# DevSinghSachan/emdr2

Measured on AMD Instinct MI355X. Metric: mips_queries_per_sec, higher is better.
Workload: dtype f16; 1 GPU; BASELINE configs[1]: MIPS-only top-50, 512 queries/search over a 21015324 x 768 fp16 index resident in HBM; rows=21015324, dim=768, top_k=50, parallelism=index row-sharded x1, all-gather(top-k) + merge, cus=256, allgather_bytes_per_rank=0

## Files before the change

### emdr2_amd/_native.py

```python
import ctypes
import os

_HERE = os.path.dirname(os.path.abspath(__file__))
LIB_PATH = os.path.join(_HERE, "lib", "libemdr2_hip.so")

EMDR2_ABI_VERSION = 4
FLAG_AMBIGUOUS = 1
FLAG_OVERFLOW = 2
MAX_TOPK = 120

_ERRORS = {-1: "bad argument", -2: "workspace too small", -3: "HIP launch/runtime error", -4: "unsupported shape"}

_vp, _i32, _i64, _sz = ctypes.c_void_p, ctypes.c_int, ctypes.c_int64, ctypes.c_size_t
SIGNATURES = {
    "emdr2_abi_version": (_i32, []),
    "emdr2_device_cu_count": (_i32, []),
    "emdr2_mips_layout_bytes": (_i32, [_i64, _i32, ctypes.POINTER(_sz)]),
    "emdr2_mips_pack_rows": (_i32, [_vp, _i64, _i32, _i64, _i64, _vp, _vp, _vp]),
    "emdr2_mips_unpack_rows": (_i32, [_vp, _i64, _i32, _vp, _i64, _vp, _vp]),
    "emdr2_mips_workspace_bytes": (_i32, [_i32, _i32, _i32, ctypes.POINTER(_sz)]),
    "emdr2_mips_search": (_i32, [_vp, _i64, _i32, _i64, _vp, _vp, _i32, _i32, _vp, _vp, _vp, _vp, _vp, _vp, _sz, _vp]),
    "emdr2_mips_exact_workspace_bytes": (_i32, [_i64, _i32, ctypes.POINTER(_sz)]),
    "emdr2_mips_search_exact": (_i32, [_vp, _i64, _i32, _i64, _vp, _i32, _vp, _i32, _i32, _vp, _vp, _vp, _vp, _vp, _vp, _sz, _vp]),
    "emdr2_mips_merge": (_i32, [_vp, _vp, _vp, _i32, _i32, _i32, _vp, _vp, _vp, _vp]),
    "emdr2_mips_search_f32": (_i32, [_vp, _i64, _i32, _i64, _vp, _vp, _i32, _i32, _vp, _vp, _vp, _vp, _vp, _vp, _sz, _vp]),
    "emdr2_mips_exact_workspace_bytes_f32": (_i32, [_i64, _i32, ctypes.POINTER(_sz)]),
    "emdr2_mips_search_exact_f32": (_i32, [_vp, _i64, _i32, _i64, _vp, _i32, _vp, _i32, _i32, _vp, _vp, _vp, _vp, _vp, _vp, _sz, _vp]),
    "emdr2_mips_merge_f32": (_i32, [_vp, _vp, _vp, _i32, _i32, _i32, _vp, _vp, _vp, _vp]),
    "emdr2_mips_search_records": (_i32, [_vp, _i64, _i32, _i64, _vp, _vp, _i32, _i32, _vp, _i32, _vp, _vp, _vp, _sz, _vp]),
    "emdr2_mips_merge_records": (_i32, [_vp, _i32, _i32, _i32, _i32, _vp, _vp, _vp, _vp]),
    "emdr2_mips_pack_records": (_i32, [_vp, _vp, _vp, _vp, _i32, _i32, _i32, _vp, _vp]),
    "emdr2_mips_shadow_bytes": (_i32, [_i64, _i32, ctypes.POINTER(_sz), ctypes.POINTER(_sz)]),
    "emdr2_mips_seal_shadow": (_i32, [_vp, _i64, _i32, _vp, _vp, _vp, _vp]),
    "emdr2_mips_search_shadow": (_i32, [_vp, _i64, _i32, _i64, _vp, _vp, _vp, _i64, _vp, _i32, _i32, _vp, _i32, _vp, _vp, _vp, _vp, _vp, _vp, _sz, _vp]),
    "emdr2_mips_shadow_launches": (_i32, []),
    "emdr2_mips_debug_scores": (_i32, [_vp, _i64, _i32, _vp, _i32, _vp, _vp, _sz, _vp]),
    "emdr2_mips_set_timing": (_i32, [_i32]),
    "emdr2_mips_timing_collect": (_i32, [ctypes.POINTER(ctypes.c_float), ctypes.POINTER(_i64), _i32, ctypes.POINTER(_i32)]),
}

SIGNATURES["emdr2_assemble_evidence"] = (_i32, [_vp, _vp, _i32, _i32, _i32, _vp, _vp, _i32, _vp, _i32, _i32, _i32, _i32, _i32,
                                                  _vp, _vp, _vp, _vp, _vp, _vp])


_f32 = ctypes.c_float
_u32 = ctypes.c_uint32
SIGNATURES["emdr2_gemm_nt_bf16"] = (_i32, [_vp, _i64, _vp, _i64, _vp, _i64, _i32, _i32, _i32, _i32, _i64, _i64, _i64, _i32, _i64, _i64, _i64,
                                             _f32, _vp, _i32, _vp, _vp, _i32, _i32, _i32, _f32, _u32, _vp])
SIGNATURES["emdr2_gemm_tn_bf16"] = (_i32, [_vp, _i64, _vp, _i64, _vp, _i64, _i32, _i32, _i32, _i32, _vp, _vp])
SIGNATURES["emdr2_dropout"] = (_i32, [_vp, _vp, _i64, _i32, _f32, _u32, _vp])
SIGNATURES["emdr2_transpose_bf16"] = (_i32, [_vp, _i64, _vp, _i64, _i32, _i32, _i32, _i64, _i64, _i32, _i64, _i64, _vp, _vp])


SIGNATURES.update({
    "emdr2_layernorm_fwd": (_i32, [_vp, _vp, _vp, _vp, _vp, _vp, _i64, _i32, _f32, _vp]),
    "emdr2_layernorm_bwd": (_i32, [_vp, _vp, _vp, _vp, _vp, _vp, _vp, _vp, _vp, _i64, _i32, _vp]),
    "emdr2_layernorm_bwd_mask": (_i32, [_vp, _vp, _vp, _vp, _vp, _vp, _vp, _vp, _vp, _i64, _i32, _vp, _f32, _u32, _vp]),
    "emdr2_softmax_mask_fwd": (_i32, [_vp, _vp, _vp, _i32, _i32, _i32, _i32, _i32, _vp, _vp, _f32, _u32, _vp]),
    "emdr2_softmax_mask_bwd": (_i32, [_vp, _vp, _vp, _vp, _vp, _vp, _i32, _i32, _i32, _i32, _i32, _f32, _u32, _vp, _vp]),
    "emdr2_softmax_mask_t": (_i32, [_vp, _vp, _vp, _vp, _vp, _vp, _vp, _i32, _i32, _i32, _i32, _i32, _f32, _u32, _vp]),
    "emdr2_gelu_bwd": (_i32, [_vp, _vp, _vp, _i64, _vp]),
    "emdr2_embedding_fwd": (_i32, [_vp, _vp, _vp, _vp, _vp, _vp, _i64, _i32, _i32, _f32, _u32, _vp]),
    "emdr2_embedding_bwd": (_i32, [_vp, _vp, _vp, _vp, _vp, _vp, _i64, _i32, _i32, _i32, _f32, _u32, _vp]),
    "emdr2_attention_fwd": (_i32, [_vp, _i64, _i64, _i64, _vp, _i64, _i64, _i64, _vp, _i64, _i64, _i64, _vp, _vp, _vp, _i32, _i32, _i32, _i32, _i32, _i32,
                                   _f32, _f32, _u32, _vp, _vp, _vp]),
    "emdr2_attention_bwd": (_i32, [_vp, _i64, _i64, _i64, _vp, _i64, _i64, _i64, _vp, _i64, _i64, _i64, _vp, _vp, _vp, _i64, _i64, _vp, _vp, _i64, _i64,
                                   _vp, _vp, _vp, _vp, _vp, _i32, _i32, _i32, _i32, _i32, _i32, _f32, _f32, _u32, _vp]),
    "emdr2_lse_gather_fwd": (_i32, [_vp, _vp, _vp, _vp, _i64, _i32, _vp]),
    "emdr2_lse_gather_bwd": (_i32, [_vp, _vp, _vp, _vp, _vp, _i64, _i32, _vp]),
    "emdr2_sumsq_f32": (_i32, [_vp, _i64, _vp, _vp, _vp]),
    "emdr2_adam_step": (_i32, [_vp, _vp, _vp, _vp, _vp, _i64, _f32, _f32, _f32, _f32, _f32, _i32, _vp, _f32, _vp]),
    "emdr2_adam_step_flat": (_i32, [_vp, _vp, _vp, _vp, _vp, _i64, _i64, _f32, _f32, _f32, _f32, _f32, _i32, _vp, _f32, _vp]),
    "emdr2_scale_cast_f32_to_bf16": (_i32, [_vp, _vp, _i64, _f32, _vp]),
    "emdr2_widen_bf16_to_f32": (_i32, [_vp, _vp, _i64, _vp]),
    "emdr2_cast_f32_to_bf16": (_i32, [_vp, _vp, _i64, _vp]),
    "emdr2_accum_bf16_to_f32": (_i32, [_vp, _vp, _i64, _f32, _vp]),
})


SIGNATURES.update({
    "emdr2_seq_lengths": (_i32, [_vp, _i32, _i32, _vp, _vp, _vp]),
    "emdr2_seq_pack_ids": (_i32, [_vp, _vp, _vp, _i32, _i32, _i64, _i64, _vp, _vp, _vp, _vp, _vp]),
    "emdr2_gather_rows": (_i32, [_vp, _vp, _vp, _i64, _i32, _vp]),
    "emdr2_scatter_rows": (_i32, [_vp, _vp, _vp, _i64, _i32, _vp]),
    "emdr2_embedding_packed_fwd": (_i32, [_vp, _vp, _vp, _vp, _vp, _vp, _vp, _i64, _i32, _i32, _f32, _u32, _vp]),
    "emdr2_embedding_packed_bwd": (_i32, [_vp, _vp, _vp, _i32, _vp, _vp, _vp, _vp, _i64, _i32, _i32, _i32, _f32, _u32, _vp]),
    "emdr2_attention_varlen_fwd": (_i32, [_vp, _i64, _i64, _i64, _vp, _i64, _i64, _i64, _vp, _i64, _i64, _i64, _vp, _vp, _vp, _vp, _vp, _i64, _i64,
                                          _i32, _i32, _i32, _i32, _i32, _i32, _f32, _f32, _u32, _vp, _vp, _vp]),
# ... 77 lines not shown
```

### emdr2_amd/csrc/mips_api.hip

```cpp
#include "../../include/emdr2_mips.h"
#include "mips_kernels.h"
#include "exp_hooks.h"
#include <stdlib.h>

namespace {

#define TIMING_SLOTS 2048
struct Timing {
    bool enabled = false;
    hipEvent_t ev[2 * TIMING_SLOTS] = {};
    int created = 0;
    int n = 0;
    int64_t rows[TIMING_SLOTS] = {};
} g_timing;

int cu_count()
{
    static int cus = 0;
    if (!cus) {
        int dev = 0;
        hipDeviceProp_t prop;
        if (hipGetDevice(&dev) != hipSuccess || hipGetDeviceProperties(&prop, dev) != hipSuccess) return 256;
        cus = prop.multiProcessorCount > 0 ? prop.multiProcessorCount : 256;
    }
    return cus;
}

inline size_t align_up(size_t x, size_t a) { return (x + a - 1) / a * a; }

#define env_int(name, dflt) EXP_ENV_INT(name, dflt)

struct Workspace {
    char *q_frag;
    char *q_tiled;
    float *qnorm, *tau;
    unsigned *count;
    uint2 *cand, *cand8;
};

size_t carve(char *base, int dim, Workspace *w)
{
    size_t off = 0;
    auto take = [&](size_t bytes) { char *p = base ? base + off : nullptr; off += align_up(bytes, 256); return p; };
    char *f = take((size_t)(dim / 32) * 512 * 64);
    char *a = take((size_t)(dim / 32) * 512 * 64);
    char *b = take(512 * sizeof(float));
    char *c = take(512 * sizeof(float));
    char *d = take((512 + 8 * 512 + 8 * (size_t)SCAN8_PROG_UINTS) * sizeof(unsigned));
    char *e = take((size_t)512 * CAPQ * sizeof(uint2));
    char *g = take((size_t)512 * 8 * SUBCAP * sizeof(uint2));
    if (w) { w->q_frag = f; w->q_tiled = a; w->qnorm = (float *)b; w->tau = (float *)c; w->count = (unsigned *)d; w->cand = (uint2 *)e; w->cand8 = (uint2 *)g; }
    return off;
}

struct Shadow {
    const void *image;
    const float *table;
    int64_t min_rows;
};
long g_shadow_launches = 0;

bool bad_shape(int64_t n_rows, int dim) { return n_rows < 0 || n_rows >= ((int64_t)1 << 31) - 1024 || dim < 64 || dim > 8192 || (dim % 32) != 0; }

}

extern "C" {

int emdr2_abi_version(void) { return EMDR2_ABI_VERSION; }

int emdr2_device_cu_count(void) { return cu_count(); }

int emdr2_mips_set_timing(int enabled)
{
    g_timing.enabled = enabled != 0;
    g_timing.n = 0;
    return EMDR2_OK;
}

int emdr2_mips_timing_collect(float *ms, int64_t *rows, int max_n, int *n_out)
{
    const int n = g_timing.n < max_n ? g_timing.n : max_n;
    for (int i = 0; i < n; ++i) {
        if (hipEventSynchronize(g_timing.ev[2 * i + 1]) != hipSuccess) return EMDR2_E_LAUNCH;
        if (hipEventElapsedTime(&ms[i], g_timing.ev[2 * i], g_timing.ev[2 * i + 1]) != hipSuccess) return EMDR2_E_LAUNCH;
        rows[i] = g_timing.rows[i];
    }
    if (n_out) *n_out = n;
    g_timing.n = 0;
    return EMDR2_OK;
}

int emdr2_mips_layout_bytes(int64_t n_rows, int dim, size_t *bytes)
{
    if (!bytes || bad_shape(n_rows, dim)) return EMDR2_E_BADARG;
    const int64_t padded = (n_rows + 511) / 512 * 512;
    *bytes = (size_t)padded * dim * 2;
    return EMDR2_OK;
}

int emdr2_mips_pack_rows(const void *rows_rm, int64_t n_chunk, int dim, int64_t row_offset, int64_t n_rows_total,
                         void *tiled, float *emax_sq, emdr2_stream_t stream)
{
    if (!rows_rm || !tiled || !emax_sq || bad_shape(n_rows_total, dim) || n_chunk < 0 || row_offset < 0 ||
        row_offset + n_chunk > n_rows_total)
        return EMDR2_E_BADARG;
    return mips_launch_pack_rows(rows_rm, n_chunk, dim, row_offset, tiled, emax_sq, (hipStream_t)stream);
}

int emdr2_mips_unpack_rows(const void *tiled, int64_t n_rows_total, int dim, const int64_t *row_ids, int64_t n_out,
                           void *rows_rm, emdr2_stream_t stream)
{
    if (!tiled || !row_ids || !rows_rm || bad_shape(n_rows_total, dim) || n_out < 0) return EMDR2_E_BADARG;
    return mips_launch_unpack_rows(tiled, dim, row_ids, n_out, rows_rm, (hipStream_t)stream);
}

int emdr2_mips_workspace_bytes(int n_q, int dim, int k, size_t *bytes)
{
    if (!bytes || n_q < 1 || k < 1 || k > EMDR2_MAX_TOPK || bad_shape(0, dim)) return EMDR2_E_BADARG;
    *bytes = carve(nullptr, dim, nullptr);
    return EMDR2_OK;
}

static int variant_for(int nq) { return nq <= 128 ? 2 : (nq <= 256 ? 1 : 0); }
static const int kBM[3] = {128, 256, 512};
static const int kBN[3] = {512, 256, 128};

static int search_impl(const void *tiled, int64_t n_rows, int dim, int64_t row_base, const float *emax_sq,
                       const void *queries, int n_q, int k, const int32_t *ids, void *out_dist, int32_t *out_idx,
                       int64_t *out_row, uint32_t *out_flags, void *workspace, size_t workspace_bytes,
                       emdr2_stream_t stream_, int f32, uint4 *out_rec = nullptr, const Shadow *shadow = nullptr)
{
    if (!tiled || !emax_sq || !queries || !out_flags || !workspace) return EMDR2_E_BADARG;
    if (!out_rec && (!out_dist || !out_idx || !out_row)) return EMDR2_E_BADARG;
    if (out_rec && ((uintptr_t)out_rec & 15)) return EMDR2_E_BADARG;
    if (n_q < 1 || k < 1 || k > EMDR2_MAX_TOPK || bad_shape(n_rows, dim) || n_rows < 1) return EMDR2_E_BADARG;
    Workspace w;
    if (carve((char *)workspace, dim, &w) > workspace_bytes) return EMDR2_E_WORKSPACE;
    hipStream_t stream = (hipStream_t)stream_;
    const int kp = k <= 56 ? 64 : 128;
    const int seg0 = env_int("EMDR2_MIPS_SEG0", 8192) / 512 * 512;
    const int growth = env_int("EMDR2_MIPS_GROWTH", 8);
    const int growth_i8 = env_int("EMDR2_MIPS_GROWTH_I8", 2);
    if (seg0 < 512 || seg0 > (int)CAPQ - 512 || growth < 2 || growth_i8 < 2) return EMDR2_E_BADARG;
    const int force_variant = env_int("EMDR2_MIPS_VARIANT", -1);
    const int cus = env_int("EMDR2_MIPS_GRID", cu_count());
    const int scan_kernel = env_int("EMDR2_MIPS_KERNEL", 1);
    const int ablate = env_int("EMDR2_MIPS_ABLATE", 0);

    for (int q0 = 0; q0 < n_q; q0 += EMDR2_MAX_QUERIES_PER_PASS) {
        const int nqp = (n_q - q0) < EMDR2_MAX_QUERIES_PER_PASS ? (n_q - q0) : EMDR2_MAX_QUERIES_PER_PASS;
        int variant = variant_for(nqp);
        if (force_variant >= 0 && force_variant <= 2 && kBN[force_variant] >= nqp) variant = force_variant;
        const int BM = kBM[variant], BN = kBN[variant];
        const uint16_t *qp = (const uint16_t *)queries + (size_t)q0 * dim;
        int rc;
        if ((rc = mips_launch_pack_queries(qp, nqp, dim, BN, w.q_tiled, w.qnorm, stream))) return rc;
        EXP_MIPS_PACK_QUERIES_FRAG(variant, scan_kernel, qp, nqp, dim, w, stream, rc)
        const int64_t dense_rows = n_rows < seg0 ? n_rows : seg0;
        unsigned *const count8 = w.count + 512, *const prog0 = count8 + 8 * 512;
        if ((rc = mips_launch_init(w.tau, w.count, out_flags + q0, BN, nqp, (unsigned)dense_rows, count8,
                                   8 * 512 + (variant == 0 ? 8 * (size_t)SCAN8_PROG_UINTS : 0), stream)))
            return rc;

        ScanParams sp;
        sp.e_tiled = (const char *)tiled;
        sp.q_tiled = w.q_tiled;
        sp.tau = w.tau;
        sp.cand = w.cand;
        sp.count = w.count;
        sp.flags = out_flags + q0;
        sp.dense_out = nullptr;
        sp.nch = dim / 32;
        sp.n_rows = (int)n_rows;
        sp.n_q = nqp;
        sp.capq = CAPQ;
        sp.cand8 = w.cand8;
        sp.count8 = count8;
        sp.dense_row0 = 0;
        sp.tune = env_int("EMDR2_MIPS_TUNE", 17);
        sp.trace = (unsigned long long *)w.cand + (size_t)511 * CAPQ;

        int scan8_launches = 0;
        const bool shadow_ok = shadow && variant <= 1 && scan_kernel == 1 && (dim % 256) == 0 && n_rows - dense_rows >= shadow->min_rows;
        char *const q8_tiled = w.q_frag;
        float *const qc = (float *)(w.q_frag + (size_t)(dim / 64) * 512 * 64);
        if (shadow_ok && (rc = mips_launch_pack_queries_i8(qp, nqp, dim, BN, q8_tiled, qc, stream))) return rc;
        const bool couple = EXP_MIPS_COUPLE();
        int64_t done = 0, seg_end = dense_rows;
        int mode = 1;
        while (done < n_rows) {
            sp.tile_begin = (int)(done / BM);
            sp.tile_end = (int)((seg_end + BM - 1) / BM);
            const int tiles = sp.tile_end - sp.tile_begin;
            const int grid = tiles < cus ? tiles : cus;
            const bool timed = g_timing.enabled && g_timing.n < TIMING_SLOTS;
            if (timed) {
                while (g_timing.created <= g_timing.n) {
                    if (hipEventCreate(&g_timing.ev[2 * g_timing.created]) != hipSuccess ||
                        hipEventCreate(&g_timing.ev[2 * g_timing.created + 1]) != hipSuccess)
                        return EMDR2_E_LAUNCH;
                    ++g_timing.created;
                }
                if (hipEventRecord(g_timing.ev[2 * g_timing.n], stream) != hipSuccess) return EMDR2_E_LAUNCH;
            }
            bool int8_segment = false;
            EXP_MIPS_SCAN_VARIANT(mode, variant, ablate, scan_kernel, sp, w, grid, seg_end, n_rows, done, stream, rc)
            {
                rc = -4;
                if (mode == 0 && variant <= 1 && scan_kernel == 1) {
                    unsigned *prog = (couple && scan8_launches < 8) ? prog0 + (size_t)SCAN8_PROG_UINTS * scan8_launches : nullptr;
                    if (shadow_ok && seg_end - done >= shadow->min_rows) {
                        rc = mips_launch_scan8i(sp, shadow->image, shadow->table, q8_tiled, qc, BN, done, seg_end, cus, prog, stream);
                        if (rc == 0) { int8_segment = true; ++g_shadow_launches; }
                    }
                    if (rc == -4) rc = mips_launch_scan8(sp, BN, done, seg_end, cus, prog, stream);
                    if (rc == 0) ++scan8_launches;
                }
                if (rc == -4) rc = mips_launch_scan(variant, mode, sp, grid, stream);
            }
            if (rc) return rc;
            if (timed) {
                if (hipEventRecord(g_timing.ev[2 * g_timing.n + 1], stream) != hipSuccess) return EMDR2_E_LAUNCH;
                g_timing.rows[g_timing.n] = seg_end - done;
                ++g_timing.n;
            }
            if (int8_segment && (rc = mips_launch_rescore(sp, qp, (unsigned)kp, stream))) return rc;
            if (seg_end < n_rows && (rc = mips_launch_select(w.cand, w.count, w.cand8, count8, w.tau, out_flags + q0, CAPQ, kp, nqp, stream))) return rc;
            done = seg_end;
            const int64_t next_boundary = done * ((shadow_ok && done * (growth_i8 - 1) >= shadow->min_rows) ? growth_i8 : growth);
            seg_end = next_boundary < n_rows ? next_boundary : n_rows;
            if (n_rows - seg_end < seg_end / 2) seg_end = n_rows;
            mode = 0;
        }

        FinalizeParams fp;
        fp.e_tiled = (const char *)tiled;
        fp.queries = qp;
        fp.cand = w.cand;
        fp.count = w.count;
        fp.cand8 = w.cand8;
        fp.count8 = count8;
        fp.tau = w.tau;
        fp.qnorm = w.qnorm;
        fp.emax_sq = emax_sq;
        fp.ids = ids;
        fp.out_rec = out_rec ? out_rec + (size_t)q0 * k : nullptr;
        fp.out_dist = out_rec ? nullptr : (f32 ? (void *)((float *)out_dist + (size_t)q0 * k) : (void *)((uint16_t *)out_dist + (size_t)q0 * k));
        fp.f32 = f32;
        fp.out_idx = out_rec ? nullptr : out_idx + (size_t)q0 * k;
        fp.out_row = out_rec ? nullptr : out_row + (size_t)q0 * k;
        fp.flags = out_flags + q0;
        fp.n_rows = n_rows;
        fp.row_base = row_base;
        fp.dim = dim;
        fp.n_q = nqp;
        fp.k = k;
        fp.kp = kp;
        fp.capq = CAPQ;
        if ((rc = mips_launch_finalize(fp, true, stream))) return rc;
    }
    return EMDR2_OK;
}

int emdr2_mips_search(const void *tiled, int64_t n_rows, int dim, int64_t row_base, const float *emax_sq,
                      const void *queries, int n_q, int k, const int32_t *ids, void *out_dist, int32_t *out_idx,
                      int64_t *out_row, uint32_t *out_flags, void *workspace, size_t workspace_bytes,
                      emdr2_stream_t stream)
{
    return search_impl(tiled, n_rows, dim, row_base, emax_sq, queries, n_q, k, ids, out_dist, out_idx, out_row, out_flags, workspace,
                       workspace_bytes, stream, 0);
}

int emdr2_mips_search_f32(const void *tiled, int64_t n_rows, int dim, int64_t row_base, const float *emax_sq,
                          const void *queries, int n_q, int k, const int32_t *ids, float *out_dist, int32_t *out_idx,
                          int64_t *out_row, uint32_t *out_flags, void *workspace, size_t workspace_bytes,
                          emdr2_stream_t stream)
{
    return search_impl(tiled, n_rows, dim, row_base, emax_sq, queries, n_q, k, ids, out_dist, out_idx, out_row, out_flags, workspace,
                       workspace_bytes, stream, 1);
}

int emdr2_mips_search_records(const void *tiled, int64_t n_rows, int dim, int64_t row_base, const float *emax_sq, const void *queries, int n_q,
                              int k, const int32_t *ids, int f32, void *out_records, uint32_t *out_flags, void *workspace,
                              size_t workspace_bytes, emdr2_stream_t stream)
{
    if (!out_records) return EMDR2_E_BADARG;
    return search_impl(tiled, n_rows, dim, row_base, emax_sq, queries, n_q, k, ids, nullptr, nullptr, nullptr, out_flags, workspace,
                       workspace_bytes, stream, f32 ? 1 : 0, (uint4 *)out_records);
}

int emdr2_mips_shadow_bytes(int64_t n_rows, int dim, size_t *image_bytes, size_t *table_bytes)
{
    if (!image_bytes || !table_bytes || bad_shape(n_rows, dim) || (dim % 256) != 0) return EMDR2_E_BADARG;
    const int64_t padded = (n_rows + 511) / 512 * 512;
    *image_bytes = (size_t)padded * dim;
    *table_bytes = (size_t)(padded / 256) * 4 * sizeof(float);
    return EMDR2_OK;
}

int emdr2_mips_seal_shadow(const void *tiled, int64_t n_rows, int dim, void *shadow, void *table, uint32_t *nonfinite, emdr2_stream_t stream)
{
    if (!tiled || !shadow || !table || !nonfinite || ((uintptr_t)table & 15) || bad_shape(n_rows, dim) || (dim % 256) != 0) return EMDR2_E_BADARG;
    return mips_launch_seal_shadow(tiled, n_rows, dim, shadow, (float *)table, nonfinite, (hipStream_t)stream);
}

int emdr2_mips_search_shadow(const void *tiled, int64_t n_rows, int dim, int64_t row_base, const float *emax_sq, const void *shadow,
                             const void *table, int64_t shadow_min_rows, const void *queries, int n_q, int k, const int32_t *ids, int f32,
                             void *out_dist, int32_t *out_idx, int64_t *out_row, void *out_records, uint32_t *out_flags, void *workspace,
                             size_t workspace_bytes, emdr2_stream_t stream)
{
    if (!shadow || !table || ((uintptr_t)table & 15) || shadow_min_rows < 1 || (dim % 256) != 0) return EMDR2_E_BADARG;
    const Shadow sh = {shadow, (const float *)table, shadow_min_rows};
    return search_impl(tiled, n_rows, dim, row_base, emax_sq, queries, n_q, k, ids, out_dist, out_idx, out_row, out_flags, workspace,
                       workspace_bytes, stream, f32 ? 1 : 0, (uint4 *)out_records, &sh);
}

int emdr2_mips_shadow_launches(void) { return (int)g_shadow_launches; }

int emdr2_mips_merge_records(const void *records_in, int n_shards, int n_q, int k, int f32, void *out_dist, int32_t *out_idx, int64_t *out_row,
                             emdr2_stream_t stream)
{
    if (!records_in || ((uintptr_t)records_in & 15) || !out_dist || !out_idx || !out_row || n_shards < 1 || n_q < 1 || k < 1) return EMDR2_E_BADARG;
    return mips_launch_merge_records((const uint4 *)records_in, n_shards, n_q, k, f32 ? 1 : 0, out_dist, out_idx, out_row, (hipStream_t)stream);
}

int emdr2_mips_pack_records(const void *dist, const int32_t *idx, const int64_t *row, const int32_t *sel, int n_sel, int k, int f32,
                            void *records, emdr2_stream_t stream)
{
    if (!dist || !idx || !row || !sel || !records || ((uintptr_t)records & 15) || n_sel < 0 || k < 1) return EMDR2_E_BADARG;
    return mips_launch_pack_records(dist, idx, row, sel, n_sel, k, f32 ? 1 : 0, (uint4 *)records, (hipStream_t)stream);
}

int emdr2_mips_exact_workspace_bytes_f32(int64_t n_rows, int n_sel, size_t *bytes)
{
    if (!bytes || n_rows < 1 || n_sel < 0) return EMDR2_E_BADARG;
    *bytes = align_up((size_t)8 * (size_t)n_rows * sizeof(uint32_t), 256);
    return EMDR2_OK;
}

int emdr2_mips_search_exact_f32(const void *tiled, int64_t n_rows, int dim, int64_t row_base, const void *queries,
                                int n_q, const int32_t *sel, int n_sel, int k, const int32_t *ids, float *out_dist,
                                int32_t *out_idx, int64_t *out_row, uint32_t *out_flags, void *workspace,
                                size_t workspace_bytes, emdr2_stream_t stream_)
{
    if (!tiled || !queries || !sel || !out_dist || !out_idx || !out_row || !out_flags || !workspace) return EMDR2_E_BADARG;
    if (n_q < 1 || n_sel < 0 || k < 1 || k > EMDR2_MAX_TOPK || bad_shape(n_rows, dim) || n_rows < 1) return EMDR2_E_BADARG;
    if (workspace_bytes < (size_t)8 * (size_t)n_rows * sizeof(uint32_t)) return EMDR2_E_WORKSPACE;
    hipStream_t stream = (hipStream_t)stream_;
    for (int b = 0; b < n_sel; b += 8) {
        const int nb = (n_sel - b) < 8 ? (n_sel - b) : 8;
        int rc;
        if ((rc = mips_launch_exact_scores_f32((const char *)tiled, n_rows, dim, (const uint16_t *)queries, sel + b, nb,
                                               (uint32_t *)workspace, stream)))
            return rc;
        if ((rc = mips_launch_exact_select_f32((const uint32_t *)workspace, n_rows, row_base, sel + b, nb, k, ids, out_dist, out_idx,
                                               out_row, out_flags, stream)))
            return rc;
    }
    return EMDR2_OK;
}

int emdr2_mips_merge_f32(const float *dist_in, const int32_t *idx_in, const int64_t *row_in, int n_shards, int n_q, int k,
                         float *out_dist, int32_t *out_idx, int64_t *out_row, emdr2_stream_t stream)
{
    if (!dist_in || !idx_in || !row_in || !out_dist || !out_idx || !out_row || n_shards < 1 || n_q < 1 || k < 1) return EMDR2_E_BADARG;
    return mips_launch_merge_f32(dist_in, idx_in, row_in, n_shards, n_q, k, out_dist, out_idx, out_row, (hipStream_t)stream);
}

int emdr2_mips_exact_workspace_bytes(int64_t n_rows, int n_sel, size_t *bytes)
{
// ... 73 lines not shown
```

### emdr2_amd/csrc/mips_kernels.h

```cpp
#pragma once
#include <hip/hip_runtime.h>
#include <stdint.h>

#define CAPQ 16384u
#define SUBCAP 1024u

struct ScanParams {
    const char *e_tiled;
    const char *q_tiled;
    const float *tau;
    uint2 *cand;
    unsigned *count;
    unsigned *flags;
    float *dense_out;
    int nch;
    int tile_begin, tile_end;
    int n_rows;
    int n_q;
    unsigned capq;
    uint2 *cand8;
    unsigned *count8;
    int dense_row0;
    int tune;
    unsigned long long *trace;
};

int mips_launch_scan(int variant, int mode, const ScanParams &p, int grid, hipStream_t stream);
#define SCAN8_PROG_UINTS (256 * 64)
int mips_launch_scan8(const ScanParams &p, int bn, int64_t row_begin, int64_t row_end, int cus, unsigned *prog, hipStream_t stream);
int mips_launch_seal_shadow(const void *tiled, int64_t n_rows, int dim, void *e8, float *blk, unsigned *nonfinite, hipStream_t stream);
int mips_launch_pack_queries_i8(const void *queries, int n_q, int dim, int bn, void *q8_tiled, float *qc, hipStream_t stream);
int mips_launch_scan8i(const ScanParams &p, const void *e8_tiled, const float *blk, const void *q8_tiled, const float *qc, int bn, int64_t row_begin,
                       int64_t row_end, int cus, unsigned *prog, hipStream_t stream);
int mips_launch_rescore(const ScanParams &p, const void *queries, unsigned pre, hipStream_t stream);
int mips_launch_scan_pp(int variant, int depth, const ScanParams &p, int grid, hipStream_t stream);
int mips_launch_scan_q8(int abl, const ScanParams &p, int grid, hipStream_t stream);
int mips_launch_pack_queries_frag(const void *queries, int n_q, int dim, void *q_frag, hipStream_t stream);
int mips_launch_scan_ablate(int abl, const ScanParams &p, int grid, hipStream_t stream);

int mips_launch_pack_rows(const void *rows_rm, int64_t n_chunk, int dim, int64_t row_offset, void *tiled,
                          float *emax_sq, hipStream_t stream);
int mips_launch_unpack_rows(const void *tiled, int dim, const int64_t *row_ids, int64_t n_out, void *rows_rm,
                            hipStream_t stream);
int mips_launch_pack_queries(const void *queries, int n_q, int dim, int bn, void *q_tiled, float *qnorm,
                             hipStream_t stream);
int mips_launch_init(float *tau, unsigned *count, unsigned *flags, int bn, int n_q, unsigned dense_count, unsigned *zero, size_t n_zero,
                     hipStream_t stream);
int mips_launch_select(uint2 *cand, unsigned *count, uint2 *cand8, unsigned *count8, float *tau, unsigned *flags, unsigned capq, int kp, int n_q,
                       hipStream_t stream);
struct FinalizeParams {
    const char *e_tiled;
    const uint16_t *queries;
    const uint2 *cand;
    const unsigned *count;
    uint2 *cand8;
    unsigned *count8;
    const float *tau;
    const float *qnorm;
    const float *emax_sq;
    const int32_t *ids;
    void *out_dist;
    int32_t *out_idx;
    int64_t *out_row;
    unsigned *flags;
    int64_t n_rows, row_base;
    int dim, n_q, k, kp;
    unsigned capq;
    int f32;
    uint4 *out_rec;
};
int mips_launch_finalize(const FinalizeParams &p, bool select_first, hipStream_t stream);
int mips_launch_merge_f32(const float *dist_in, const int32_t *idx_in, const int64_t *row_in, int n_shards, int n_q, int k,
                          float *out_dist, int32_t *out_idx, int64_t *out_row, hipStream_t stream);
int mips_launch_merge_records(const uint4 *rec_in, int n_shards, int n_q, int k, int f32, void *out_dist, int32_t *out_idx, int64_t *out_row,
                              hipStream_t stream);
int mips_launch_pack_records(const void *dist, const int32_t *idx, const int64_t *row, const int32_t *sel, int n_sel, int k, int f32, uint4 *rec,
                             hipStream_t stream);
int mips_launch_merge(const uint16_t *dist_in, const int32_t *idx_in, const int64_t *row_in, int n_shards, int n_q,
                      int k, uint16_t *out_dist, int32_t *out_idx, int64_t *out_row, hipStream_t stream);

int mips_launch_exact_scores(const char *e_tiled, int64_t n_rows, int dim, const uint16_t *queries,
                             const int32_t *sel, int n_sel, uint16_t *hkeys ,
                             hipStream_t stream);
int mips_launch_exact_select(const uint16_t *hkeys, int64_t n_rows, int64_t row_base, const int32_t *sel, int n_sel,
                             int k, const int32_t *ids, uint16_t *out_dist, int32_t *out_idx, int64_t *out_row,
// ... 7 lines not shown
```

### emdr2_amd/csrc/mips_scan8i.hip

```cpp
#include "mips_device.h"
#include "mips_kernels.h"

namespace {

typedef int intx4 __attribute__((ext_vector_type(4)));

#define S8_BUF 65536
#define S8_SLOT 16384
#define S8_QCAP 2040
#define S8_WCAP 255
#define S8_FLUSH_AT 128

struct Scan8Params {
    ScanParams s;
    int t_begin, t_end;
    int halves;
    int bn;
    int last_stripe;
    int total, per;
    unsigned *prog;
    const float4 *blk;
    const float4 *qc;
};

__device__ __forceinline__ int s8i_theta(float tau, float t, float a, float b, float s, float n, float d)
{
    if (tau == __builtin_inff()) return 0x7fffffff;
    const float ts = t * s;
    if (!(ts > 0.f)) return (int)0x80000000;
    const float eps = (a * n + b * d) * 1.0001f;
    float num = tau - eps;
    num -= fabsf(num) * 1e-6f;
    float x = num * __builtin_amdgcn_rcpf(ts);
    x -= fabsf(x) * 1e-5f;
    x = floorf(x) - 1.f;
    if (!(x > -2.0e9f)) return (int)0x80000000;
    if (x > 2.0e9f) return 0x7fffffff;
    return (int)x;
}

__device__ __forceinline__ void s8_append(const ScanParams &p, unsigned xcc, unsigned q, unsigned score_bits, unsigned row)
{
    const unsigned slot = __hip_atomic_fetch_add(&p.count8[xcc * 512 + q], 1u, __ATOMIC_RELAXED, __HIP_MEMORY_SCOPE_WORKGROUP);
    if (slot < SUBCAP) { p.cand8[((size_t)q * 8 + xcc) * SUBCAP + slot] = make_uint2(score_bits, row); return; }
    const unsigned s2 = __hip_atomic_fetch_add(&p.count[q], 1u, __ATOMIC_RELAXED, __HIP_MEMORY_SCOPE_AGENT);
    if (s2 < p.capq) p.cand[(size_t)q * p.capq + s2] = make_uint2(score_bits, row);
}

__device__ __forceinline__ void s8_flush(const ScanParams &p, const char *qbuf, const unsigned *cnt, int tid, unsigned xcc)
{
    const int region = tid >> 6;
    unsigned m = ((const volatile __attribute__((address_space(3))) unsigned *)cnt)[region];
    if (m > S8_WCAP) m = S8_WCAP;
    for (unsigned i = tid & 63; i < m; i += 64) {
        const uint4 e = ((const uint4 *)qbuf)[region * S8_WCAP + i];
        s8_append(p, xcc, e.z, e.x, e.y);
    }
}

__global__ void __launch_bounds__(512) mips_scan8i_kernel(Scan8Params P)
{
    extern __shared__ __attribute__((aligned(16))) char smem[];
    const ScanParams &p = P.s;
    char *const qbuf = smem + 2 * S8_BUF;
    unsigned *const qcnt = (unsigned *)(qbuf + S8_QCAP * 16);
    const int tid = threadIdx.x, lane = tid & 63;
    const int wave = __builtin_amdgcn_readfirstlane(tid >> 6);
    const int wr = wave >> 2, wc = wave & 3;
    const int l31 = lane & 31, hi = lane >> 5;

    const int xcd = blockIdx.x & 7, slot = blockIdx.x >> 3, wg_per_xcd = gridDim.x >> 3;
    const int seq_lo = xcd * P.per;
    int seq_hi = seq_lo + P.per; if (seq_hi > P.total) seq_hi = P.total;
    const int first = seq_lo + slot;
    if (first >= seq_hi) return;
    const int my_count = (seq_hi - first + wg_per_xcd - 1) / wg_per_xcd;
    const int KT = p.nch >> 1;
    unsigned *const flagw = qcnt + 8;
    if (tid < 8) qcnt[tid] = 0;
    if (tid == 0) *flagw = 0;
    unsigned wq = 0;
    const unsigned xcc = __builtin_amdgcn_s_getreg(20 | (0 << 6) | (3 << 11)) & 7u;
    const int hq = P.halves == 2 ? first & 1 : 0;
    float4 qcv[4];
    float tauv[4];
#pragma unroll
    for (int qt = 0; qt < 4; ++qt) {
        const int q = hq * 256 + wc * 64 + qt * 16 + ((lane & 3) * 4 + ((lane & 15) >> 2));
        tauv[qt] = q < p.n_q ? p.tau[q] : __builtin_inff();
        qcv[qt] = P.qc[q < p.n_q ? q : 0];
    }

    const int ja = (wave >> 2) & 1, qa = wave & 3;
    const int jb = (wave >> 1) & 1, qb = wave & 1;
    const uint32_t offA = (uint32_t)(ja * STRIPE_CHUNK_BYTES + qa * 1024 + lane * 16);
    const uint32_t q_stage = (uint32_t)P.bn * 64;
    const uint32_t offB = (uint32_t)(jb * q_stage + ((wave >> 2) * 64) * 64 + qb * 1024 + lane * 16);
    int s_i = 0, s_kt = 0;
    const char *sA0, *sA1, *sB;
    auto cursor_item = [&](int i) {
// ... 412 lines not shown
```

### include/emdr2_mips.h

```cpp
#ifndef EMDR2_MIPS_H
#define EMDR2_MIPS_H

#include <stddef.h>
#include <stdint.h>

#ifdef __cplusplus
extern "C" {
#endif

#define EMDR2_ABI_VERSION 4

#define EMDR2_OK 0
#define EMDR2_E_BADARG (-1)
#define EMDR2_E_WORKSPACE (-2)
#define EMDR2_E_LAUNCH (-3)
#define EMDR2_E_UNSUPPORTED (-4)

#define EMDR2_FLAG_AMBIGUOUS 1u
#define EMDR2_FLAG_OVERFLOW 2u

#define EMDR2_STRIPE_ROWS 128
#define EMDR2_CHUNK_K 32
#define EMDR2_MAX_TOPK 120
#define EMDR2_MAX_QUERIES_PER_PASS 512
// ... 9 lines not shown
int emdr2_mips_pack_rows(const void *rows_rm, int64_t n_chunk, int dim, int64_t row_offset,
                         int64_t n_rows_total, void *tiled, float *emax_sq, emdr2_stream_t stream);

int emdr2_mips_unpack_rows(const void *tiled, int64_t n_rows_total, int dim, const int64_t *row_ids,
                           int64_t n_out, void *rows_rm, emdr2_stream_t stream);

int emdr2_mips_workspace_bytes(int n_q, int dim, int k, size_t *bytes);

int emdr2_mips_search(const void *tiled, int64_t n_rows, int dim, int64_t row_base, const float *emax_sq,
                      const void *queries, int n_q, int k, const int32_t *ids,
                      void *out_dist, int32_t *out_idx, int64_t *out_row, uint32_t *out_flags,
                      void *workspace, size_t workspace_bytes, emdr2_stream_t stream);

int emdr2_mips_exact_workspace_bytes(int64_t n_rows, int n_sel, size_t *bytes);

int emdr2_mips_search_exact(const void *tiled, int64_t n_rows, int dim, int64_t row_base,
                            const void *queries, int n_q, const int32_t *sel, int n_sel, int k,
                            const int32_t *ids, void *out_dist, int32_t *out_idx, int64_t *out_row,
                            uint32_t *out_flags, void *workspace, size_t workspace_bytes,
                            emdr2_stream_t stream);

int emdr2_mips_merge(const void *dist_in, const int32_t *idx_in, const int64_t *row_in, int n_shards,
                     int n_q, int k, void *out_dist, int32_t *out_idx, int64_t *out_row,
                     emdr2_stream_t stream);

int emdr2_mips_search_f32(const void *tiled, int64_t n_rows, int dim, int64_t row_base, const float *emax_sq,
                          const void *queries, int n_q, int k, const int32_t *ids,
                          float *out_dist, int32_t *out_idx, int64_t *out_row, uint32_t *out_flags,
                          void *workspace, size_t workspace_bytes, emdr2_stream_t stream);
int emdr2_mips_exact_workspace_bytes_f32(int64_t n_rows, int n_sel, size_t *bytes);
int emdr2_mips_search_exact_f32(const void *tiled, int64_t n_rows, int dim, int64_t row_base, const void *queries, int n_q,
                                const int32_t *sel, int n_sel, int k, const int32_t *ids, float *out_dist, int32_t *out_idx,
                                int64_t *out_row, uint32_t *out_flags, void *workspace, size_t workspace_bytes,
                                emdr2_stream_t stream);
int emdr2_mips_merge_f32(const float *dist_in, const int32_t *idx_in, const int64_t *row_in, int n_shards, int n_q, int k,
                         float *out_dist, int32_t *out_idx, int64_t *out_row, emdr2_stream_t stream);


int emdr2_mips_search_records(const void *tiled, int64_t n_rows, int dim, int64_t row_base, const float *emax_sq, const void *queries, int n_q,
                              int k, const int32_t *ids, int f32, void *out_records, uint32_t *out_flags, void *workspace,
                              size_t workspace_bytes, emdr2_stream_t stream);
int emdr2_mips_merge_records(const void *records_in, int n_shards, int n_q, int k, int f32, void *out_dist, int32_t *out_idx, int64_t *out_row,
                             emdr2_stream_t stream);
int emdr2_mips_pack_records(const void *dist, const int32_t *idx, const int64_t *row, const int32_t *sel, int n_sel, int k, int f32,
                            void *records, emdr2_stream_t stream);

int emdr2_mips_shadow_bytes(int64_t n_rows, int dim, size_t *image_bytes, size_t *table_bytes);
int emdr2_mips_seal_shadow(const void *tiled, int64_t n_rows, int dim, void *shadow, void *table, uint32_t *nonfinite, emdr2_stream_t stream);
int emdr2_mips_search_shadow(const void *tiled, int64_t n_rows, int dim, int64_t row_base, const float *emax_sq, const void *shadow,
                             const void *table, int64_t shadow_min_rows, const void *queries, int n_q, int k, const int32_t *ids, int f32,
                             void *out_dist, int32_t *out_idx, int64_t *out_row, void *out_records, uint32_t *out_flags, void *workspace,
                             size_t workspace_bytes, emdr2_stream_t stream);
int emdr2_mips_shadow_launches(void);

int emdr2_mips_debug_scores(const void *tiled, int64_t n_rows, int dim, const void *queries, int n_q,
                            float *out_scores, void *workspace, size_t workspace_bytes,
                            emdr2_stream_t stream);

int emdr2_mips_set_timing(int enabled);
int emdr2_mips_timing_collect(float *ms, int64_t *rows, int max_n, int *n_out);

#ifdef __cplusplus
}
#endif
#endif
```

Before: 60850 queries/s.

## Add register-resident int8 shadow scan kernel with query fragments held in VGPRs

Adds a new int8 shadow scan kernel that loads every query fragment for all chunks into registers once per workgroup. Index stripes are then streamed into LDS through a multi-chunk global_load_lds pipeline, which removes the repeated per-stripe query reloads of the existing scan8i kernel. It is enabled by default through an environment switch and falls back to scan8i when the shape is unsupported. The trade is heavy register use (bq arrays sized by chunk count) and larger LDS, which may lower occupancy or cause spills for dim 768 (12 chunks).

```diff
diff --git a/emdr2_amd/_native.py b/emdr2_amd/_native.py
--- a/emdr2_amd/_native.py
+++ b/emdr2_amd/_native.py
@@ -34,6 +34,7 @@
     "emdr2_mips_seal_shadow": (_i32, [_vp, _i64, _i32, _vp, _vp, _vp, _vp]),
     "emdr2_mips_search_shadow": (_i32, [_vp, _i64, _i32, _i64, _vp, _vp, _vp, _i64, _vp, _i32, _i32, _vp, _i32, _vp, _vp, _vp, _vp, _vp, _vp, _sz, _vp]),
     "emdr2_mips_shadow_launches": (_i32, []),
+    "emdr2_mips_shadow_resident_launches": (_i32, []),
     "emdr2_mips_debug_scores": (_i32, [_vp, _i64, _i32, _vp, _i32, _vp, _vp, _sz, _vp]),
     "emdr2_mips_set_timing": (_i32, [_i32]),
     "emdr2_mips_timing_collect": (_i32, [ctypes.POINTER(ctypes.c_float), ctypes.POINTER(_i64), _i32, ctypes.POINTER(_i32)]),
diff --git a/emdr2_amd/csrc/mips_api.hip b/emdr2_amd/csrc/mips_api.hip
--- a/emdr2_amd/csrc/mips_api.hip
+++ b/emdr2_amd/csrc/mips_api.hip
@@ -59,6 +59,7 @@
     int64_t min_rows;
 };
 long g_shadow_launches = 0;
+long g_shadow_resident_launches = 0;
 
 bool bad_shape(int64_t n_rows, int dim) { return n_rows < 0 || n_rows >= ((int64_t)1 << 31) - 1024 || dim < 64 || dim > 8192 || (dim % 32) != 0; }
 
@@ -146,6 +147,7 @@
     const int cus = env_int("EMDR2_MIPS_GRID", cu_count());
     const int scan_kernel = env_int("EMDR2_MIPS_KERNEL", 1);
     const int ablate = env_int("EMDR2_MIPS_ABLATE", 0);
+    const bool i8_resident = env_int("EMDR2_MIPS_I8_RESIDENT", 1) != 0;
 
     for (int q0 = 0; q0 < n_q; q0 += EMDR2_MAX_QUERIES_PER_PASS) {
         const int nqp = (n_q - q0) < EMDR2_MAX_QUERIES_PER_PASS ? (n_q - q0) : EMDR2_MAX_QUERIES_PER_PASS;
@@ -210,7 +212,11 @@
                 if (mode == 0 && variant <= 1 && scan_kernel == 1) {
                     unsigned *prog = (couple && scan8_launches < 8) ? prog0 + (size_t)SCAN8_PROG_UINTS * scan8_launches : nullptr;
                     if (shadow_ok && seg_end - done >= shadow->min_rows) {
-                        rc = mips_launch_scan8i(sp, shadow->image, shadow->table, q8_tiled, qc, BN, done, seg_end, cus, prog, stream);
+                        if (i8_resident) {
+                            rc = mips_launch_scan8r(sp, shadow->image, shadow->table, q8_tiled, qc, BN, done, seg_end, cus, prog, stream);
+                            if (rc == 0) ++g_shadow_resident_launches;
+                        }
+                        if (rc == -4) rc = mips_launch_scan8i(sp, shadow->image, shadow->table, q8_tiled, qc, BN, done, seg_end, cus, prog, stream);
                         if (rc == 0) { int8_segment = true; ++g_shadow_launches; }
                     }
                     if (rc == -4) rc = mips_launch_scan8(sp, BN, done, seg_end, cus, prog, stream);
@@ -316,6 +322,8 @@
 }
 
 int emdr2_mips_shadow_launches(void) { return (int)g_shadow_launches; }
+
+int emdr2_mips_shadow_resident_launches(void) { return (int)g_shadow_resident_launches; }
 
 int emdr2_mips_merge_records(const void *records_in, int n_shards, int n_q, int k, int f32, void *out_dist, int32_t *out_idx, int64_t *out_row,
                              emdr2_stream_t stream)
diff --git a/emdr2_amd/csrc/mips_kernels.h b/emdr2_amd/csrc/mips_kernels.h
--- a/emdr2_amd/csrc/mips_kernels.h
+++ b/emdr2_amd/csrc/mips_kernels.h
@@ -31,6 +31,8 @@
 int mips_launch_seal_shadow(const void *tiled, int64_t n_rows, int dim, void *e8, float *blk, unsigned *nonfinite, hipStream_t stream);
 int mips_launch_pack_queries_i8(const void *queries, int n_q, int dim, int bn, void *q8_tiled, float *qc, hipStream_t stream);
 int mips_launch_scan8i(const ScanParams &p, const void *e8_tiled, const float *blk, const void *q8_tiled, const float *qc, int bn, int64_t row_begin,
+                       int64_t row_end, int cus, unsigned *prog, hipStream_t stream);
+int mips_launch_scan8r(const ScanParams &p, const void *e8_tiled, const float *blk, const void *q8_tiled, const float *qc, int bn, int64_t row_begin,
                        int64_t row_end, int cus, unsigned *prog, hipStream_t stream);
 int mips_launch_rescore(const ScanParams &p, const void *queries, unsigned pre, hipStream_t stream);
 int mips_launch_scan_pp(int variant, int depth, const ScanParams &p, int grid, hipStream_t stream);
diff --git a/emdr2_amd/csrc/mips_scan8i.hip b/emdr2_amd/csrc/mips_scan8i.hip
--- a/emdr2_amd/csrc/mips_scan8i.hip
+++ b/emdr2_amd/csrc/mips_scan8i.hip
@@ -1,9 +1,7 @@
 #include "mips_device.h"
-#include "mips_kernels.h"
+#include "mips_scan8i_common.h"
 
 namespace {
-
-typedef int intx4 __attribute__((ext_vector_type(4)));
 
 #define S8_BUF 65536
 #define S8_SLOT 16384
@@ -11,41 +9,6 @@
 #define S8_WCAP 255
 #define S8_FLUSH_AT 128
 
-struct Scan8Params {
-    ScanParams s;
-    int t_begin, t_end;
-    int halves;
-    int bn;
-    int last_stripe;
-    int total, per;
-    unsigned *prog;
-    const float4 *blk;
-    const float4 *qc;
-};
-
-__device__ __forceinline__ int s8i_theta(float tau, float t, float a, float b, float s, float n, float d)
-{
-    if (tau == __builtin_inff()) return 0x7fffffff;
-    const float ts = t * s;
-    if (!(ts > 0.f)) return (int)0x80000000;
-    const float eps = (a * n + b * d) * 1.0001f;
-    float num = tau - eps;
-    num -= fabsf(num) * 1e-6f;
-    float x = num * __builtin_amdgcn_rcpf(ts);
-    x -= fabsf(x) * 1e-5f;
-    x = floorf(x) - 1.f;
-    if (!(x > -2.0e9f)) return (int)0x80000000;
-    if (x > 2.0e9f) return 0x7fffffff;
-    return (int)x;
-}
-
-__device__ __forceinline__ void s8_append(const ScanParams &p, unsigned xcc, unsigned q, unsigned score_bits, unsigned row)
-{
-    const unsigned slot = __hip_atomic_fetch_add(&p.count8[xcc * 512 + q], 1u, __ATOMIC_RELAXED, __HIP_MEMORY_SCOPE_WORKGROUP);
-    if (slot < SUBCAP) { p.cand8[((size_t)q * 8 + xcc) * SUBCAP + slot] = make_uint2(score_bits, row); return; }
-    const unsigned s2 = __hip_atomic_fetch_add(&p.count[q], 1u, __ATOMIC_RELAXED, __HIP_MEMORY_SCOPE_AGENT);
-    if (s2 < p.capq) p.cand[(size_t)q * p.capq + s2] = make_uint2(score_bits, row);
-}
 
 __device__ __forceinline__ void s8_flush(const ScanParams &p, const char *qbuf, const unsigned *cnt, int tid, unsigned xcc)
 {
diff --git a/emdr2_amd/csrc/mips_scan8i_common.h b/emdr2_amd/csrc/mips_scan8i_common.h
--- /dev/null
+++ b/emdr2_amd/csrc/mips_scan8i_common.h
@@ -0,0 +1,45 @@
+#pragma once
+#include "mips_device.h"
+#include "mips_kernels.h"
+
+namespace {
+
+typedef int intx4 __attribute__((ext_vector_type(4)));
+
+struct Scan8Params {
+    ScanParams s;
+    int t_begin, t_end;
+    int halves;
+    int bn;
+    int last_stripe;
+    int total, per;
+    unsigned *prog;
+    const float4 *blk;
+    const float4 *qc;
+};
+
+__device__ __forceinline__ int s8i_theta(float tau, float t, float a, float b, float s, float n, float d)
+{
+    if (tau == __builtin_inff()) return 0x7fffffff;
+    const float ts = t * s;
+    if (!(ts > 0.f)) return (int)0x80000000;
+    const float eps = (a * n + b * d) * 1.0001f;
+    float num = tau - eps;
+    num -= fabsf(num) * 1e-6f;
+    float x = num * __builtin_amdgcn_rcpf(ts);
+    x -= fabsf(x) * 1e-5f;
+    x = floorf(x) - 1.f;
+    if (!(x > -2.0e9f)) return (int)0x80000000;
+    if (x > 2.0e9f) return 0x7fffffff;
+    return (int)x;
+}
+
+__device__ __forceinline__ void s8_append(const ScanParams &p, unsigned xcc, unsigned q, unsigned score_bits, unsigned row)
+{
+    const unsigned slot = __hip_atomic_fetch_add(&p.count8[xcc * 512 + q], 1u, __ATOMIC_RELAXED, __HIP_MEMORY_SCOPE_WORKGROUP);
+    if (slot < SUBCAP) { p.cand8[((size_t)q * 8 + xcc) * SUBCAP + slot] = make_uint2(score_bits, row); return; }
+    const unsigned s2 = __hip_atomic_fetch_add(&p.count[q], 1u, __ATOMIC_RELAXED, __HIP_MEMORY_SCOPE_AGENT);
+    if (s2 < p.capq) p.cand[(size_t)q * p.capq + s2] = make_uint2(score_bits, row);
+}
+
+}
diff --git a/emdr2_amd/csrc/mips_scan8r.hip b/emdr2_amd/csrc/mips_scan8r.hip
--- /dev/null
+++ b/emdr2_amd/csrc/mips_scan8r.hip
@@ -0,0 +1,260 @@
+#include "mips_scan8i_common.h"
+
+namespace {
+
+#define R8_CHUNK 8192
+#define R8_QCAP 2040
+#define R8_WCAP 510
+#define R8_FLUSH_AT 256
+
+__device__ __forceinline__ void r8_flush(const ScanParams &p, const char *qbuf, const unsigned *cnt, int tid, unsigned xcc)
+{
+    const int region = tid >> 6;
+    unsigned m = ((const volatile __attribute__((address_space(3))) unsigned *)cnt)[region];
+    if (m > R8_WCAP) m = R8_WCAP;
+    for (unsigned i = tid & 63; i < m; i += 64) {
+        const uint4 e = ((const uint4 *)qbuf)[region * R8_WCAP + i];
+        s8_append(p, xcc, e.z, e.x, e.y);
+    }
+}
+
+template <int NCH>
+__global__ void __launch_bounds__(256) mips_scan8r_kernel(Scan8Params P)
+{
+    extern __shared__ __attribute__((aligned(16))) char smem[];
+    const ScanParams &p = P.s;
+    char *const qbuf = smem + NCH * R8_CHUNK;
+    unsigned *const qcnt = (unsigned *)(qbuf + R8_QCAP * 16);
+    float4 *const qtab = (float4 *)(qbuf + R8_QCAP * 16 + 128);
+    const int tid = threadIdx.x, lane = tid & 63;
+    const int wave = __builtin_amdgcn_readfirstlane(tid >> 6);
+
+    const int xcd = blockIdx.x & 7, slot = blockIdx.x >> 3, wg_per_xcd = gridDim.x >> 3;
+    const int seq_lo = xcd * P.per;
+    int seq_hi = seq_lo + P.per; if (seq_hi > P.total) seq_hi = P.total;
+    const int first = seq_lo + slot;
+    if (first >= seq_hi) return;
+    const int my_count = (seq_hi - first + wg_per_xcd - 1) / wg_per_xcd;
+    unsigned *const flagw = qcnt + 8;
+    if (tid < 4) qcnt[tid] = 0;
+    if (tid == 0) *flagw = 0;
+    unsigned wq = 0;
+    const unsigned xcc = __builtin_amdgcn_s_getreg(20 | (0 << 6) | (3 << 11)) & 7u;
+    const int hq = P.halves == 2 ? first & 1 : 0;
+
+    const int l15 = lane & 15, lq = lane >> 4;
+    const int prow = (l15 & 3) * 4 + (l15 >> 2);
+    const int frag_rd = prow * 64 + ((lq ^ ((prow >> 2) & 3)) << 4);
+
+    intx4 bq[NCH][4];
+    {
+        const char *qb = p.q_tiled + (size_t)(hq * 256 + wave * 64) * 64 + frag_rd;
+#pragma unroll
+        for (int c = 0; c < NCH; ++c)
+#pragma unroll
+            for (int qt = 0; qt < 4; ++qt) bq[c][qt] = *(const intx4 *)(qb + (size_t)c * P.bn * 64 + qt * 1024);
+    }
+    {
+        const int q = hq * 256 + tid;
+        float4 v = P.qc[q < p.n_q ? q : 0];
+        v.w = q < p.n_q ? p.tau[q] : __builtin_inff();
+        qtab[tid] = v;
+    }
+    asm volatile("s_waitcnt vmcnt(0)" ::: "memory");
+    __builtin_amdgcn_sched_barrier(0);
+
+    const uint32_t piece = (uint32_t)(wave * 2048 + lane * 16);
+    auto stripe_src = [&](int i) {
+        if (i >= my_count) i = my_count - 1;
+        const int pos = first + i * wg_per_xcd;
+        int st = P.t_begin + (P.halves == 2 ? pos >> 1 : pos);
+        if (st > P.last_stripe) st = P.last_stripe;
+        return p.e_tiled + (size_t)st * (NCH * R8_CHUNK);
+    };
+    const char *cur = stripe_src(0), *nxt = stripe_src(1);
+#define R8_STAGE(SRC, C)                                                                                                                  \
+    do {                                                                                                                                  \
+        const char *s_ = (SRC) + (C) * R8_CHUNK + piece;                                                                                        \
+        char *d_ = smem + (C) * R8_CHUNK + wave * 2048;                                                                                   \
+        __builtin_amdgcn_global_load_lds((gptr_t *)s_, (lptr_t *)d_, 16, 0, 0);                                                           \
+        __builtin_amdgcn_global_load_lds((gptr_t *)(s_ + 1024), (lptr_t *)(d_ + 1024), 16, 0, 0);                                         \
+    } while (0)
+#define R8_BARRIER()                                                                                                                      \
+    __builtin_amdgcn_s_barrier();                                                                                                         \
+    __builtin_amdgcn_sched_barrier(0)
+#define R8_WAIT(N) asm volatile("s_waitcnt vmcnt(%0)" ::"n"(N) : "memory")
+    intx4 av[2][8];
+#define R8_READ_A(C)                                                                                                                      \
+    _Pragma("unroll") for (int rt = 0; rt < 8; ++rt)                                                                                      \
+        av[(C) & 1][rt] = *(const intx4 *)(smem + (C) * R8_CHUNK + rt * 1024 + frag_rd)
+
+    auto maybe_flush = [&]() {
+        unsigned n_ = 0;
+#pragma unroll
+        for (int w = 0; w < 4; ++w) n_ = max(n_, ((const volatile __attribute__((address_space(3))) unsigned *)qcnt)[w]);
+        if (n_ >= R8_FLUSH_AT) {
+            r8_flush(p, qbuf, qcnt, tid, xcc);
+            asm volatile("s_waitcnt vmcnt(0)" ::: "memory");
+            R8_BARRIER();
+            if (tid < 4) qcnt[tid] = 0;
+            wq = 0;
+            R8_BARRIER();
+        }
+    };
+
+    unsigned *const prog = (P.prog && P.halves == 2) ? P.prog + (xcd * (wg_per_xcd >> 1) + (slot >> 1)) * 64 : nullptr;
+    int ticks = 0;
+#define R8_COUPLE()                                                                                                                       \
+    if (prog && wave == 0) {                                                                                                              \
+        const int tot_ = __builtin_amdgcn_readfirstlane((int)*(volatile __attribute__((address_space(3))) unsigned *)flagw);               \
+        if (lane == 0) {                                                                                                                  \
+            atomicAdd(prog, 1u);                                                                                                          \
+            __builtin_amdgcn_global_load_lds((gptr_t *)prog, (lptr_t *)flagw, 4, 0, 16);         \
+        }                                                                                                                                 \
+        const int lead_ = 2 * ticks - tot_;                              \
+        ++ticks;                                                                                                                          \
+        if (!(P.s.tune & 64)) for (int i_ = 0; i_ < (lead_ > 6 ? 6 : lead_) - 1; ++i_) __builtin_amdgcn_s_sleep(16);      \
+    }
+
+    intx4 acc[8][4];
+    const intx4 zero4 = {0, 0, 0, 0};
+
+#pragma unroll
+    for (int c = 0; c < NCH - 1; ++c) R8_STAGE(cur, c);
+    R8_WAIT(2 * (NCH - 2));
+    __builtin_amdgcn_sched_barrier(0);
+    R8_BARRIER();
+    R8_READ_A(0);
+
+    for (int ti = 0; ti < my_count; ++ti) {
+#pragma unroll
+        for (int c = 0; c < NCH; ++c) {
+            R8_WAIT(2 * (NCH - 3));
+            __builtin_amdgcn_sched_barrier(0);
+            R8_BARRIER();
+            if (c == 0) {
+                if (ti > 0) maybe_flush();
+                R8_STAGE(cur, NCH - 1);
+            } else {
+                R8_STAGE(nxt, c - 1);
+            }
+            __builtin_amdgcn_sched_barrier(0);
+            R8_READ_A((c + 1) % NCH);
+#pragma unroll
+            for (int rt = 0; rt < 8; ++rt)
+#pragma unroll
+                for (int qt = 0; qt < 4; ++qt)
+                    acc[rt][qt] = __builtin_amdgcn_mfma_i32_16x16x64_i8(av[c & 1][rt], bq[c][qt], c == 0 ? zero4 : acc[rt][qt], 0, 0, 0);
+            __builtin_amdgcn_sched_group_barrier(0x008, 4, 0);
+#pragma unroll
+            for (int g = 0; g < 4; ++g) {
+                __builtin_amdgcn_sched_group_barrier(0x100, 2, 0);
+                __builtin_amdgcn_sched_group_barrier(0x008, 4, 0);
+            }
+            __builtin_amdgcn_sched_group_barrier(0x008, 12, 0);
+            __builtin_amdgcn_sched_barrier(0);
+            if ((c & 3) == 3) { R8_COUPLE(); }
+        }
+
+        const int pos = first + ti * wg_per_xcd;
+        const int stripe = P.t_begin + (P.halves == 2 ? pos >> 1 : pos);
+        cur = nxt; nxt = stripe_src(ti + 2);
+        const int elane = (int)__builtin_amdgcn_mbcnt_hi(~0u, __builtin_amdgcn_mbcnt_lo(~0u, 0u));
+        const int e15 = elane & 15, eq = elane >> 4;
+        const int row_w = stripe * 128 + eq;
+        const bool tail = (stripe + 1) * 128 > p.n_rows;
+        bool stored = false;
+        const __attribute__((address_space(4))) float *bk = (const __attribute__((address_space(4))) float *)(uintptr_t)(P.blk + (stripe >> 1));
+        const float bs = bk[0], bn_ = bk[1], bd = bk[2];
+#pragma unroll
+        for (int qt = 0; qt < 4; ++qt) {
+            const unsigned q = (unsigned)(hq * 256 + wave * 64 + qt * 16 + (e15 & 3) * 4 + (e15 >> 2));
+            float4 qcv;
+            asm volatile("ds_read_b128 %0, %1\n\ts_waitcnt lgkmcnt(0)" : "=v"(qcv) : "v"((unsigned)(uintptr_t)qtab + (q & 255u) * 16u) : "memory");
+            const int tau = s8i_theta(qcv.w, qcv.x, qcv.y, qcv.z, bs, bn_, bd);
+            int mr[8];
+#pragma unroll
+            for (int rt = 0; rt < 8; ++rt) mr[rt] = max(max(acc[rt][qt][0], acc[rt][qt][1]), max(acc[rt][qt][2], acc[rt][qt][3]));
+            const int m = max(max(max(mr[0], mr[1]), max(mr[2], mr[3])), max(max(mr[4], mr[5]), max(mr[6], mr[7])));
+            if (__builtin_amdgcn_ballot_w64(m >= tau) == 0) continue;
+#pragma unroll
+            for (int rt = 0; rt < 8; ++rt) {
+                if (__builtin_amdgcn_ballot_w64(mr[rt] >= tau) == 0) continue;
+#pragma unroll
+                for (int r = 0; r < 4; ++r) {
+                    const int v = acc[rt][qt][r];
+                    const int row = row_w + rt * 16 + 4 * r;
+                    const unsigned long long mask = __builtin_amdgcn_ballot_w64((v >= tau) && (!tail || row < p.n_rows));
+                    if (mask == 0) continue;
+                    if ((mask >> elane) & 1ull) {
+                        const unsigned mine = wq + __builtin_amdgcn_mbcnt_hi((unsigned)(mask >> 32), __builtin_amdgcn_mbcnt_lo((unsigned)mask, 0));
+                        if (mine < R8_WCAP) {
+                            ((uint2 *)qbuf)[2 * (wave * R8_WCAP + mine)] = make_uint2((unsigned)v, (unsigned)row);
+                            ((unsigned *)qbuf)[4 * (wave * R8_WCAP + mine) + 2] = q;
+                        } else {
+                            s8_append(p, xcc, q, (unsigned)v, (unsigned)row);
+                            stored = true;
+                        }
+                    }
+                    wq += (unsigned)__popcll(mask);
+                }
+            }
+        }
+        if (__builtin_amdgcn_ballot_w64(stored)) asm volatile("s_waitcnt vmcnt(0)" ::: "memory");
+        if (wq > R8_WCAP) wq = R8_WCAP;
+        if (elane == 0) qcnt[wave] = wq;
+        asm volatile("s_waitcnt lgkmcnt(0)" ::: "memory");
+        __builtin_amdgcn_sched_barrier(0);
+    }
+    if (prog && tid == 0) atomicAdd(prog, 1u << 20);
+    asm volatile("s_waitcnt vmcnt(0)" ::: "memory");
+    R8_BARRIER();
+    r8_flush(p, qbuf, qcnt, tid, xcc);
+}
+
+template <int NCH>
+int launch_r(const Scan8Params &P, int grid, hipStream_t stream)
+{
+    constexpr int LDS = NCH * R8_CHUNK + R8_QCAP * 16 + 128 + 256 * 16;
+    static bool attr_done = false;
+    if (!attr_done) {
+        if (hipFuncSetAttribute((const void *)mips_scan8r_kernel<NCH>, hipFuncAttributeMaxDynamicSharedMemorySize, LDS) != hipSuccess) return -3;
+        attr_done = true;
+    }
+    hipLaunchKernelGGL(mips_scan8r_kernel<NCH>, dim3(grid), dim3(256), LDS, stream, P);
+    return hipGetLastError() == hipSuccess ? 0 : -3;
+}
+
+}
+
+int mips_launch_scan8r(const ScanParams &p, const void *e8_tiled, const float *blk, const void *q8_tiled, const float *qc, int bn, int64_t row_begin,
+                       int64_t row_end, int cus, unsigned *prog, hipStream_t stream)
+{
+    const int nch8 = p.nch / 2;
+    if ((bn != 256 && bn != 512) || (p.nch & 1) || (nch8 != 4 && nch8 != 8 && nch8 != 12) || (row_begin & (STRIPE_ROWS - 1)) || row_end <= row_begin ||
+        row_end > p.n_rows || !p.cand8 || !p.count8)
+        return -4;
+    Scan8Params P;
+    P.s = p;
+    P.s.e_tiled = (const char *)e8_tiled;
+    P.s.q_tiled = (const char *)q8_tiled;
+    P.s.nch = nch8;
+    P.blk = (const float4 *)blk;
+    P.qc = (const float4 *)qc;
+    P.prog = prog;
+    P.bn = bn; P.halves = bn / 256;
+    P.t_begin = (int)(row_begin / STRIPE_ROWS);
+    P.t_end = (int)((row_end + STRIPE_ROWS - 1) / STRIPE_ROWS);
+    P.last_stripe = (int)((p.n_rows + STRIPE_ROWS - 1) / STRIPE_ROWS) - 1;
+    P.total = (P.t_end - P.t_begin) * P.halves;
+    int grid = cus & ~15;
+    if (grid < 16) grid = 16;
+    if (P.total < grid) return -4;
+    P.per = ((P.total + 7) >> 3);
+    P.per = (P.per + 1) & ~1;
+    switch (nch8) {
+    case 4: return launch_r<4>(P, grid, stream);
+    case 8: return launch_r<8>(P, grid, stream);
+    default: return launch_r<12>(P, grid, stream);
+    }
+}
diff --git a/include/emdr2_mips.h b/include/emdr2_mips.h
--- a/include/emdr2_mips.h
+++ b/include/emdr2_mips.h
@@ -85,6 +85,7 @@
                              void *out_dist, int32_t *out_idx, int64_t *out_row, void *out_records, uint32_t *out_flags, void *workspace,
                              size_t workspace_bytes, emdr2_stream_t stream);
 int emdr2_mips_shadow_launches(void);
+int emdr2_mips_shadow_resident_launches(void);
 
 int emdr2_mips_debug_scores(const void *tiled, int64_t n_rows, int dim, const void *queries, int n_q,
                             float *out_scores, void *workspace, size_t workspace_bytes,
```

Result: slower. 52630 queries/s (-13.5%).
